# meiji163/bokego

Hardware: AMD Instinct MI355X
Metric: leaf-evals/sec (policy+value, batched 9x9 positions) (higher is better)
Workload: dtype f32; 1 GPU; configs[1]: batch=4096 9x9 positions, PolicyNet logits+softmax and ValueNet, device-resident inputs/outputs; batch_per_gpu=4096, weights=policy_19 + value_synth (tests/golden), precision=f32

## Files before the change

bokego_amd/csrc/bk_engine.cpp:

```cpp
#include <hip/hip_runtime.h>
#include <dlfcn.h>

#include <algorithm>
#include <cmath>
#include <cstdio>
#include <cstdlib>
#include <cstring>
#include <atomic>
#include <chrono>
#include <condition_variable>
#include <mutex>
#include <new>
#include <string>
#include <thread>
#include <vector>

#include "../../include/bokego_amd.h"
#include "../../include/bokego_tree.h"
#include "bk_internal.h"

namespace {

thread_local std::string g_create_error;

// ... 158 lines not shown
    int64_t next_ticket = 1;
    std::string err;
    bk_stats_t st{};
    bool profiling = false;
    std::mutex ev_m;
    struct TimedLaunch { hipEvent_t start, stop; double host_ms; bool ticket; };
    std::vector<TimedLaunch> ev_ring;
    size_t ev_head = 0, ev_pending = 0;
    hipEvent_t epoch = nullptr;
    std::chrono::steady_clock::time_point epoch_host;
    unsigned int* h_redo = nullptr;
    unsigned int* h_redo_dev = nullptr;
    unsigned int redo_seen[BK_DEV_FLAGS] = {};
    bk_plan_opts plan;
    int no_direct = 0, no_head_part = 0, encode_overlap = 0, copy_threads = 6, no_fuse_encode = 0;
    int direct_rows = 1024;
#ifdef BK_TEST_HOOKS
    int fault_at = 0, fault_seen = 0, fault_submit = 0, coop_fault = 0;
#endif
    unsigned int* d_dev_flag = nullptr;
    unsigned int dev_seq = 0;
    float* d_coop_xchg = nullptr;
    unsigned int* d_coop_sync = nullptr;
    unsigned long long* d_stamps = nullptr;
};

namespace {

int fail(bk_engine* e, int code, const std::string& msg) {
    if (e) e->err = msg; else g_create_error = msg;
// ... 9 lines not shown
inline bool inject_fault(bk_engine*) { return false; }
#endif
inline void bump(uint64_t& c, uint64_t v = 1) { __atomic_fetch_add(&c, v, __ATOMIC_RELAXED); }
#define HIP_TRY(e, call)                                                                       \
    do {                                                                                       \
        hipError_t _s = inject_fault(e) ? hipErrorUnknown : (call);                            \
        if (_s != hipSuccess)                                                                  \
            return fail(e, _s == hipErrorOutOfMemory ? BK_ERR_OOM : BK_ERR_HIP,                \
                        std::string(#call) + ": " + hipGetErrorString(_s));                    \
    } while (0)

bool trunk_ok(const bk_trunk_weights& t) {
    for (int l = 0; l < 7; ++l)
        if (!t.conv_w[l] || !t.conv_b[l] || !t.bn_w[l] || !t.bn_b[l] || !t.bn_mean[l] || !t.bn_var[l]) return false;
    return t.head_w && t.head_b;
}

void pack_trunk(const bk_trunk_weights& t, std::vector<float>& wfrag, std::vector<float>& bias) {
    wfrag.assign(BK_WFRAG_FLOATS + BK_WFRAG_PAD_FLOATS, 0.f);
    bias.assign(7 * 128, 0.f);
    size_t base = 0;
    for (int l = 0; l < 7; ++l) {
        const int K = l == 0 ? 5 : 3, cin = l == 0 ? 27 : 128, G = l == 0 ? 2 : 8, TAPS = K * K;
        std::vector<double> scale(128);
        for (int co = 0; co < 128; ++co) scale[co] = (double)t.bn_w[l][co] / std::sqrt((double)t.bn_var[l][co] + kBnEps);
        auto out_ch = [&](int slot) { return l == 6 ? slot : bk_slot_perm(slot); };
        for (int sl = 0; sl < 128; ++sl) {
            const int co = out_ch(sl);
            bias[l * 128 + sl] = (float)(((double)t.conv_b[l][co] - (double)t.bn_mean[l][co]) * scale[co] + (double)t.bn_b[l][co]);
        }
        for (int tp = 0; tp < TAPS; ++tp)
            for (int g = 0; g < G; ++g)
                for (int ct = 0; ct < 8; ++ct)
                    for (int lane = 0; lane < 64; ++lane)
                        for (int j = 0; j < 4; ++j) {
                            const int co = out_ch(16 * ct + (lane & 15)), kq = lane >> 4;
                            int ci = bk_slot_perm(16 * g + 4 * kq + j);
                            if (l == 0 && g == 1) ci = j < 2 ? ci : (j == 2 && kq < 3 ? 24 + kq : cin);
                            float v = 0.f;
                            if (ci < cin) v = (float)((double)t.conv_w[l][((size_t)co * cin + ci) * TAPS + tp] * scale[co]);
                            wfrag[base + ((((size_t)tp * G + g) * 8 + ct) * 64 + lane) * 4 + j] = v;
                        }
        base += (size_t)TAPS * G * 2048;
    }
}

constexpr float kSa16 = 16.f;
void pack_trunk16(const bk_trunk_weights& t, std::vector<_Float16>& wfrag, std::vector<float>& bias16, float* cscale) {
    wfrag.assign(BK16_WFRAG_HALFS + BK16_WFRAG_PAD_HALFS, (_Float16)0.f);
    bias16.assign(7 * 128, 0.f);
    size_t base = 0;
    for (int l = 0; l < 7; ++l) {
        const int K = l == 0 ? 5 : 3, cin = l == 0 ? 27 : 128, S = l == 0 ? 2 : 8, TAPS = K * K;
// ... 29 lines not shown
}

template <typename T>
int upload(bk_engine* e, const std::vector<T>& h, const T** out, std::vector<void*>& fresh) {
    void* d = nullptr;
    HIP_TRY(e, hipMalloc(&d, h.size() * sizeof(T)));
    fresh.push_back(d);
    HIP_TRY(e, hipMemcpy(d, h.data(), h.size() * sizeof(T), hipMemcpyHostToDevice));
    *out = static_cast<const T*>(d);
    return BK_OK;
}

int setup_trunk(bk_engine* e, const bk_trunk_weights& t, bk_net_params& np, double head_scale, double head_shift, std::vector<void*>& fresh) {
    std::vector<float> wfrag, bias, hw(128), hb(81);
    pack_trunk(t, wfrag, bias);
    for (int c = 0; c < 128; ++c) hw[c] = (float)((double)t.head_w[c] * head_scale);
    for (int q = 0; q < 81; ++q) hb[q] = (float)((double)t.head_b[q] * head_scale + head_shift);
    std::vector<_Float16> w16;
    std::vector<float> b16;
    pack_trunk16(t, w16, b16, np.cscale16);
    np.inv_sa16 = 1.f / kSa16;
    int rc;
    if ((rc = upload(e, wfrag, &np.wfrag, fresh))) return rc;
    if ((rc = upload(e, bias, &np.bias, fresh))) return rc;
    if ((rc = upload(e, hw, &np.head_w, fresh))) return rc;
    if ((rc = upload(e, hb, &np.head_b, fresh))) return rc;
    if ((rc = upload(e, w16, &np.wfrag16, fresh))) return rc;
    if ((rc = upload(e, b16, &np.bias16, fresh))) return rc;
    return BK_OK;
}
// ... 165 lines not shown
    }
    return pl;
}

int enqueue(bk_engine* e, const void* d_feats, int dtype, int B, int n_policy, int want, float* d_logits,
            float* d_probs, float* d_values, hipStream_t stream, int precision, unsigned int* d_flag,
            unsigned int tag = 1, bool gated_redo = false, bool allow_coop = false, int lo = 0, int hi = -1) {
    if (B == 0) return BK_OK;
    if (hi < 0) hi = B;
    const bool whole = lo == 0 && hi == B;
    bk_eval_args a{};
    a.net[0] = e->net[0];
    a.net[1] = e->net[1];
    a.feats = d_feats;
    a.feats_dtype = dtype;
    const int np_all = (want & (BK_WANT_LOGITS | BK_WANT_PROBS)) ? n_policy : 0;
    a.off_p = std::min(lo, np_all);
    a.B_policy = std::min(hi, np_all);
    a.off_v = (want & BK_WANT_VALUE) ? lo : 0;
    a.B_value = (want & BK_WANT_VALUE) ? hi : 0;
    a.logits = (want & BK_WANT_LOGITS) ? d_logits : nullptr;
    a.probs = (want & BK_WANT_PROBS) ? d_probs : nullptr;
    a.values = (want & BK_WANT_VALUE) ? d_values : nullptr;
    const int cnt_p = a.B_policy - a.off_p, cnt_v = a.B_value - a.off_v;
    if (cnt_p + cnt_v == 0) return BK_OK;
#ifdef BK_STAMPS
    a.stamps = e->d_stamps;
#endif
    bool timed = false;
    size_t slot = 0;
// ... 100 lines not shown
    if (!e) return fail(nullptr, BK_ERR_OOM, "host allocation failed");
    e->device = device_id;
    e->max_batch = max_batch;
    e->has_policy = policy != nullptr;
    e->has_value = value != nullptr;
    e->precision = BK_PRECISION_F32;
    if (const char* pz = env_str("BK_PRECISION")) e->precision = std::string(pz) == "f16x2" ? BK_PRECISION_F16X2 : BK_PRECISION_F32;
    e->plan.force_nb = env_int("BK_FORCE_NB", 0);
    e->plan.no_split = env_str("BK_NO_SPLIT") != nullptr;
    e->plan.coop = env_int("BK_COOP", -1);
    e->plan.coop3 = env_int("BK_COOP3", -1);
    e->no_direct = env_str("BK_NO_DIRECT") != nullptr;
    e->no_head_part = env_str("BK_NO_HEAD_PART") != nullptr;
    e->encode_overlap = env_str("BK_ENCODE_OVERLAP") != nullptr;
    e->no_fuse_encode = env_str("BK_NO_FUSE_ENCODE") != nullptr;
    e->direct_rows = env_int("BK_DIRECT_ROWS", 1024);
    e->copy_threads = env_int("BK_COPY_THREADS", 6);
    (void)roctx();
    int rc = BK_OK;
    auto bail = [&](int code) {
        g_create_error = e->err;
        bk_engine_destroy(e);
        return code;
    };
#define TRY_CREATE(call)                                                        \
    do {                                                                        \
        hipError_t _s = (call);                                                 \
        if (_s != hipSuccess) {                                                 \
            e->err = std::string(#call) + ": " + hipGetErrorString(_s);         \
            return bail(_s == hipErrorOutOfMemory ? BK_ERR_OOM : BK_ERR_HIP);   \
// ... 430 lines not shown
                exe = bk_mfma_flop_per_workgroup(3) * (pl.head_p + pl.head_v) +
                      bk_mfma_flop_per_workgroup(pl.tail_nb) * (wgs(n_policy - 3 * pl.head_p, pl.tail_nb) + wgs(n_value - 3 * pl.head_v, pl.tail_nb));
                launches = 2;
            } else {
                exe = bk_mfma_flop_per_workgroup(pl.nb1) * (wgs(n_policy, pl.nb1) + wgs(n_value, pl.nb1));
                launches = 1;
            }
        }
    }
    if (executed_mfma_flop) *executed_mfma_flop = exe;
    if (algorithmic_flop) *algorithmic_flop = alg;
    if (n_launches) *n_launches = launches;
    return BK_OK;
}

int bk_has_test_hooks(void) {
#ifdef BK_TEST_HOOKS
    return 1;
#else
    return 0;
#endif
}

namespace {
int* option_field(bk_engine* e, const std::string& n) {
    if (n == "force_nb") return &e->plan.force_nb;
    if (n == "no_split") return &e->plan.no_split;
    if (n == "coop") return &e->plan.coop;
    if (n == "coop3") return &e->plan.coop3;
    if (n == "no_direct") return &e->no_direct;
    if (n == "no_head_part") return &e->no_head_part;
    if (n == "encode_overlap") return &e->encode_overlap;
    if (n == "no_fuse_encode") return &e->no_fuse_encode;
    if (n == "direct_rows") return &e->direct_rows;
    if (n == "copy_threads") return &e->copy_threads;
#ifdef BK_TEST_HOOKS
    if (n == "coop_fault") return &e->coop_fault;
    if (n == "fault_submit") return &e->fault_submit;
#endif
    return nullptr;
}
}

int bk_engine_set_option(bk_engine* e, const char* name, int value) {
    if (!e || !name) return BK_ERR_ARG;
    int* f = option_field(e, name);
    if (!f) return fail(e, BK_ERR_ARG, std::string("unknown engine option '") + name + "'");
    const std::string n = name;
// ... 64 lines not shown
```

bokego_amd/csrc/bk_internal.h:

```cpp
#pragma once
#include <hip/hip_runtime.h>
#include <stdint.h>

#define BK_L0_FLOATS (25 * 2 * 2048)
#define BK_L3_FLOATS (9 * 8 * 2048)
#define BK_WFRAG_FLOATS (BK_L0_FLOATS + 6 * BK_L3_FLOATS)
#define BK_WFRAG_PAD_FLOATS 16384

#define BK16_L0_STEPS 52
#define BK16_L0_HALFS (BK16_L0_STEPS * 4096)
#define BK16_L3_HALFS (72 * 4096)
#define BK16_WFRAG_HALFS (BK16_L0_HALFS + 6 * BK16_L3_HALFS)
#define BK16_WFRAG_PAD_HALFS (4 * 4096)

#define BK_PRECISION_F32 0
#define BK_PRECISION_F16X2 1

#define BK_FEATS_F32_ 0
#define BK_FEATS_U8_ 1
#define BK_FEATS_POS_ 2

struct bk_net_params {
    const float* wfrag;
    const float* bias;
    const float* head_w;
    const float* head_b;
    const float* lin1_wt;
    const float* lin1_b;
    const float* lin2_w;
    float lin2_b;
    const _Float16* wfrag16;
    const float* bias16;
    float cscale16[7];
    float inv_sa16;
};

struct bk_eval_args {
    bk_net_params net[2];
    const void* feats;
    int feats_dtype;
    int B_policy;
    int B_value;
    int off_p, off_v;
    int tasks_p, tasks_v;
    float* logits;
    float* probs;
    float* values;
    unsigned int* overflow;
    unsigned int overflow_tag;
    unsigned int* gate;
    unsigned int* gate_counter;
    unsigned int gate_tag;
    int gate_count;
    float* coop_xchg;
    unsigned int* coop_sync;
    unsigned int* coop_err;
    unsigned int coop_tag;
    int coop_fault;
    unsigned long long* stamps;
// ... 42 lines not shown
```

bokego_amd/csrc/bk_kernels.hip:

```cpp
#include <hip/hip_runtime.h>
#include <stdint.h>
#include <stdlib.h>

#include <type_traits>
#include <utility>

#include "bk_encode_dev.h"
#include "bk_internal.h"

typedef float f32x16 __attribute__((ext_vector_type(16)));
typedef float f32x4 __attribute__((ext_vector_type(4)));
typedef unsigned int u32x4 __attribute__((ext_vector_type(4)));
typedef __attribute__((address_space(3))) const char lds_cchar;
typedef __attribute__((address_space(3))) const f32x4 lds_cf32x4;


#ifndef BK_EXP
#define BK_EXP 0
#endif
#ifdef BK_STAMPS
#define STAMP(k)                                                                                   \
    do {                                                                                           \
        __builtin_amdgcn_sched_barrier(0);                                                         \
        unsigned long long _t;                                                                     \
// ... 54 lines not shown
}
template <int NB>
struct Tiles {
    static_assert(NB >= 1 && NB <= 3, "tiles are laid out for 1-, 2- and 3-board workgroups");
    static constexpr int WM = NB == 3 ? 2 : 1;
    static constexpr int WN = 8 / WM;
    static constexpr int RT = NB == 3 ? 8 : NB == 2 ? 11 : 6;
    static constexpr int CTW = 8 / WN;
    static constexpr int A0 = NB == 3 ? 1 : NB == 2 ? 2 : 0, A1 = NB == 3 ? 6 : NB == 2 ? 9 : 4;
    static constexpr int X0 = NB == 1 ? -1 : 0, X1 = NB == 2 ? 1 : -1;
    static constexpr int Y0a = NB == 3 ? 6 : NB == 2 ? 9 : 4, Y0b = NB == 3 ? 8 : NB == 2 ? 10 : 5, Y1 = NB == 2 ? 10 : NB == 1 ? 5 : -1;
    static constexpr bool WM_EDGES = NB == 3;
    static constexpr bool FRONT = false;
    static constexpr bool DB2 = NB != 3;
    static constexpr int RING = 4;
};
struct TileRow { int b, y, x; bool valid; };
template <int NB>
constexpr TileRow tile_row(int wm, int rt, int p16) {
    TileRow r{0, 4, 0, true};
    if constexpr (NB == 1) {
        if (rt <= 2) {
            const int i = rt * 16 + p16;
            r.y = 1 + i / 7; r.x = 1 + i % 7;
        } else if (rt == 3) {
            if (p16 < 14) { r.y = 1 + p16 % 7; r.x = p16 < 7 ? 0 : 8; }
            else if (p16 == 14) { r.y = 7; r.x = 7; }
            else r.valid = false;
        } else {
            if (p16 < 9) { r.y = rt == 4 ? 0 : 8; r.x = p16; } else r.valid = false;
// ... 38 lines not shown
        for (int rt = 0; rt < Tiles<NB>::RT; ++rt)
            for (int p = 0; p < 16; ++p) {
                const TileRow r = tile_row<NB>(wm, rt, p);
                const int i = (wm * Tiles<NB>::RT + rt) * 16 + p;
                t.a0[i] = Geo<NB>::addr0(r.b, r.y, r.x) - 2 * RP0 - 2 * REC0;
                t.a3v[i] = (Geo<NB>::addr3(r.b, r.y, r.x) - RP3 - REC3) | (r.valid ? 1 : 0);
            }
    return t;
}
template <int NB>
__device__ const RowTable<NB> g_rows = make_row_table<NB>();
__device__ __forceinline__ int in_slot(int c) {
    return c < 24 ? (c & ~15) | ((c & 1) << 3) | (c & 4) | (((c >> 3) & 1) << 1) | ((c >> 1) & 1) : 16 + 4 * (c - 24) + 2;
}

template <class F, bool FIRST>
__device__ __forceinline__ void conv_layer(const char* actb, const float* __restrict__ wl, f32x4 (&acc)[F::CTW][F::RT], int lane,
                                           int wm, int tile0, lds_cchar* (&ap)[F::RT], f32x4 (&W)[F::RING][F::CTW]) {
    constexpr int RT = F::RT, CTW = F::CTW, RING = F::RING;
    static_assert(RING == 4 || RING == 8, "layer 0's 50 groups leave the ring at slot 2: what the 3x3 layers start from");
    constexpr int PH = FIRST ? 0 : 50 % RING;
    constexpr int KW = FIRST ? 5 : 3, TAPS = KW * KW;
    constexpr int HALF = FIRST ? 12 : 5;
    constexpr int G = FIRST ? 2 : 8;
    constexpr int REC = FIRST ? REC0 : REC3, RP = FIRST ? RP0 : RP3;
    (void)actb;
    f32x4 part[CTW][RT];
#pragma unroll
    for (int rt = 0; rt < RT; ++rt) {
#pragma unroll
        for (int ct = 0; ct < CTW; ++ct) acc[ct][rt] = f32x4{0.f, 0.f, 0.f, 0.f};
    }

    const __amdgpu_buffer_rsrc_t wr = __builtin_amdgcn_make_buffer_rsrc(const_cast<float*>(wl + tile0 * 256), 0, 0x7ffffff0, 0x00020000);
// ... 10 lines not shown
        boff += 8192;
    };
    f32x4 A0[RT], A1[RT];
    auto read_a = [&](f32x4& dst, int rt, int imm) {
#if BK_EXP & 1
        (void)dst; (void)rt; (void)imm;
#else
        dst = *reinterpret_cast<lds_cf32x4*>(ap[rt] + imm);
#endif
    };
#if BK_EXP & 1
#pragma unroll
    for (int rt = 0; rt < RT; ++rt) { A0[rt] = f32x4{1.f, 2.f, 3.f, 4.f} * (float)lane; A1[rt] = f32x4{.5f, .25f, .125f, 1.f} * (float)lane; }
#endif

    auto do_group = [&](auto DBc, auto GIc, f32x4 (&Wc)[CTW], f32x4 (&Wn)[CTW], int delta, bool sx0, bool sx1, bool sy0, bool sy1) {
        constexpr bool DB = decltype(DBc)::value;
        constexpr int g = decltype(GIc)::value;
        constexpr int JN = (FIRST && g == 1) ? 3 : 4;
        f32x4 (&Ac)[RT] = (DB && (g & 1)) ? A1 : A0;
        f32x4 (&An)[RT] = (DB && !(g & 1)) ? A1 : A0;
        auto mfmas = [&](int j0, int j1, auto T0, auto T1, auto&& after) {
#pragma unroll
            for (int j = j0; j < j1; ++j)
#pragma unroll
                for (int rt = decltype(T0)::value; rt < decltype(T1)::value; ++rt) {
#pragma unroll
                    for (int ct = 0; ct < CTW; ++ct)
                        acc[ct][rt] = __builtin_amdgcn_mfma_f32_16x16x4f32(Wc[ct][j], Ac[rt][j], acc[ct][rt], 0, 0, 0);
                    after(j, rt);
                }
        };
        auto next_a = [&](int rt) {
            if (g == G - 1) {
// ... 45 lines not shown
            if constexpr (F::X0 >= 0) range(!sx0, std::integral_constant<int, F::X0>{}, std::integral_constant<int, F::X0 + 1>{});
            if constexpr (F::X1 >= 0) range(!sx1, std::integral_constant<int, F::X1>{}, std::integral_constant<int, F::X1 + 1>{});
            if constexpr (F::Y0a >= 0) range(!sy0, std::integral_constant<int, F::Y0a>{}, std::integral_constant<int, F::Y0b>{});
            if constexpr (F::Y1 >= 0) range(!sy1, std::integral_constant<int, F::Y1>{}, std::integral_constant<int, F::Y1 + 1>{});
            next_a(prev);
        }
    };
    using I0 = std::integral_constant<int, 0>;
    using I1 = std::integral_constant<int, 1>;
    using I2 = std::integral_constant<int, 2>;
    using I3 = std::integral_constant<int, 3>;
    using I4 = std::integral_constant<int, 4>;
    using I5 = std::integral_constant<int, 5>;
    using I6 = std::integral_constant<int, 6>;
    using I7 = std::integral_constant<int, 7>;
    auto tap = [&](auto DBc, auto PHc, int t) {
        const int ky = t / KW, kx = t - ky * KW;
        const int d = t == TAPS - 1 ? 0 : (kx == KW - 1 ? RP - (KW - 1) * REC : REC);
        const bool lo_x = kx < KW / 2, hi_x = kx > KW / 2, lo_y = ky < KW / 2, hi_y = ky > KW / 2;
        const bool sx0 = F::WM_EDGES ? (wm == 0 ? lo_x : hi_x) : lo_x, sx1 = hi_x;
        const bool sy0 = F::WM_EDGES ? (wm == 0 ? lo_y : hi_y) : lo_y, sy1 = hi_y;
        constexpr int P0 = decltype(PHc)::value;
        auto grp = [&](auto GIc) {
            constexpr int g = decltype(GIc)::value;
            do_group(DBc, GIc, W[(P0 + g) % RING], W[(P0 + g + RING - 1) % RING], d, sx0, sx1, sy0, sy1);
        };
        grp(I0{});
        grp(I1{});
        if constexpr (!FIRST) {
            grp(I2{});
            grp(I3{});
            grp(I4{});
            grp(I5{});
            grp(I6{});
            grp(I7{});
        }
    };

#pragma unroll
    for (int rt = 0; rt < RT; ++rt) read_a(A0[rt], rt, 0);
    auto taps = [&](auto DBc, int t0, int t1) {
        if constexpr (FIRST) {
            constexpr int U = RING / 2;
#pragma unroll 1
            for (int t = t0; t < t1; t += U) {
                tap(DBc, std::integral_constant<int, 0>{}, t);
                tap(DBc, std::integral_constant<int, 2>{}, t + 1);
                if constexpr (U == 4) {
                    tap(DBc, std::integral_constant<int, 4>{}, t + 2);
                    tap(DBc, std::integral_constant<int, 6>{}, t + 3);
                }
            }
        } else {
#pragma unroll 1
            for (int t = t0; t < t1; ++t) tap(DBc, std::integral_constant<int, PH>{}, t);
        }
    };
    static_assert(!FIRST || (HALF % (RING / 2) == 0 && (TAPS - 1) % (RING / 2) == 0), "layer 0: 12 + 12 taps in whole turns, then tap 24 at slot 0");
    taps(std::true_type{}, 0, HALF);
#pragma unroll
    for (int rt = 0; rt < RT; ++rt)
#pragma unroll
        for (int ct = 0; ct < CTW; ++ct) {
            part[ct][rt] = acc[ct][rt];
            acc[ct][rt] = f32x4{0.f, 0.f, 0.f, 0.f};
        }
    using DB2 = std::integral_constant<bool, F::DB2>;
    taps(DB2{}, HALF, FIRST ? TAPS - 1 : TAPS);
    if constexpr (FIRST) tap(DB2{}, std::integral_constant<int, 0>{}, TAPS - 1);
#pragma unroll
    for (int rt = 0; rt < RT; ++rt) {
        ap[rt] -= (KW - 1) * (RP + REC);
#pragma unroll
        for (int ct = 0; ct < CTW; ++ct) acc[ct][rt] = part[ct][rt] + acc[ct][rt];
    }
}

template <class F>
__device__ __forceinline__ void store_layer(char* actb, const f32x4 (&acc)[F::CTW][F::RT],
                                                 const f32x4 (&bv)[F::CTW], lds_cchar* const (&ap)[F::RT], int store_c,
                                                 unsigned valid, int dummy_byte) {
#pragma unroll
    for (int rt = 0; rt < F::RT; ++rt) {
        typedef __attribute__((address_space(3))) char lds_char;
// ... 10 lines not shown
template <class F>
__device__ __forceinline__ void load_bias(f32x4 (&bv)[F::CTW], const float* __restrict__ bias, int wn, int kq) {
#pragma unroll
    for (int ct = 0; ct < F::CTW; ++ct) bv[ct] = *reinterpret_cast<const f32x4*>(bias + 16 * (F::CTW * wn + ct) + 4 * kq);
}

__device__ __forceinline__ float wave_max(float v) {
#pragma unroll
    for (int o = 32; o > 0; o >>= 1) v = fmaxf(v, __shfl_xor(v, o, 64));
    return v;
}
__device__ __forceinline__ float wave_sum(float v) {
#pragma unroll
    for (int o = 32; o > 0; o >>= 1) v += __shfl_xor(v, o, 64);
    return v;
}

template <int NB, int THREADS>
__device__ __forceinline__ void stage_positions(const bk_eval_args& a, char* actb, int b0, int nb, int tid) {
    using G = Geo<NB>;
    static_assert(THREADS >= 256, "the encoder's mapping: one thread per board point of up to three boards");
    constexpr int SCRATCH = (G::L0_BYTES + 15) & ~15;
    static_assert(SCRATCH + (int)sizeof(bk_enc::EncLds) <= G::L3_BYTES, "the encoder's records live behind the layer-0 input");
    bk_enc::EncLds& S = *reinterpret_cast<bk_enc::EncLds*>(actb + SCRATCH);
    for (int i = tid; i < G::L0_BYTES / 16; i += THREADS) reinterpret_cast<f32x4*>(actb)[i] = f32x4{0.f, 0.f, 0.f, 0.f};
    unsigned char v[27];
    bool live;
    int p, q;
    bk_enc::encode_points(static_cast<const unsigned char*>(a.feats) + (size_t)b0 * BK_POS_BYTES, nb, tid, S, v, live, p, q);
    if (live) {
        const int y = q / 9, x = q - 9 * y;
        char* rec = actb + G::addr0(p, y, x);
#pragma unroll
        for (int c = 0; c < 27; ++c) *reinterpret_cast<float*>(rec + in_slot(c) * 4) = (float)v[c];
    }
}

template <int NB, int THREADS>
__device__ __forceinline__ void stage_input(const bk_eval_args& a, char* actb, int b0, int nb, int tid) {
    using G = Geo<NB>;
    if (a.feats_dtype == BK_FEATS_POS_) {
        stage_positions<NB, THREADS>(a, actb, b0, nb, tid);
        return;
    }
    constexpr int PER = (NB * 2187 + THREADS - 1) / THREADS;
    const int n = nb * 2187;
    float v[PER];
    if (a.feats_dtype == BK_FEATS_F32_) {
        const float* X = static_cast<const float*>(a.feats) + (size_t)b0 * 2187;
// ... 2 lines not shown
            const int e = tid + THREADS * k;
            v[k] = __builtin_nontemporal_load(X + (e < n ? e : 0));
        }
    } else {
        const uint8_t* X = static_cast<const uint8_t*>(a.feats) + (size_t)b0 * 2187;
        uint8_t raw[PER];
#pragma unroll
        for (int k = 0; k < PER; ++k) {
            const int e = tid + THREADS * k;
            raw[k] = __builtin_nontemporal_load(X + (e < n ? e : 0));
        }
#pragma unroll
        for (int k = 0; k < PER; ++k) v[k] = (float)raw[k];
    }
    STAMP_T(t_issued);
    for (int i = tid; i < G::L0_BYTES / 16; i += THREADS) reinterpret_cast<f32x4*>(actb)[i] = f32x4{0.f, 0.f, 0.f, 0.f};
    STAMP_T(t_zeroed);
    __syncthreads();
    STAMP_T(t_barrier);
#pragma unroll
    for (int k = 0; k < PER; ++k) {
        const int e = tid + THREADS * k;
        if (e < n) {
            const int b = e / 2187, ee = e - b * 2187, c = ee / 81, q = ee - c * 81, y = q / 9, x = q - 9 * y;
            *reinterpret_cast<float*>(actb + G::addr0(b, y, x) + in_slot(c) * 4) = v[k];
        }
    }
    STAMP_T(t_scattered);
#ifdef BK_STAMPS
    if (a.stamps && (tid & 63) == 0 && (tid >> 6) < 4)
        a.stamps[((size_t)blockIdx.x * 4 + (tid >> 6)) * 32 + 31] = ((t_zeroed - t_issued) & 0xffff) | (((t_barrier - t_zeroed) & 0xffff) << 16) |
                                                                   (((t_scattered - t_barrier) & 0xffff) << 32);
#endif
}

template <class G>
__device__ __forceinline__ void run_heads(const bk_eval_args& a, const bk_net_params& P, const char* actb, float* hv,
                                              int net, int lane, int board, int bg) {
    float s[2];
#pragma unroll
    for (int k = 0; k < 2; ++k) {
        const int q = lane + 64 * k;
// ... 77 lines not shown

    STAMP(0);
    using F = Tiles<NB>;
    const int wm = wave / F::WN, wn = wave - wm * F::WN;
    f32x4 Wr[F::RING][F::CTW];
    {
        const __amdgpu_buffer_rsrc_t wr0 = __builtin_amdgcn_make_buffer_rsrc(const_cast<float*>(P.wfrag + wn * F::CTW * 256), 0, 0x7ffffff0, 0x00020000);
#pragma unroll
        for (int n = 0; n < F::RING - 1; ++n)
#pragma unroll
            for (int ct = 0; ct < F::CTW; ++ct)
                Wr[n][ct] = __builtin_bit_cast(f32x4, __builtin_amdgcn_raw_buffer_load_b128(wr0, lane * 16 + ct * 1024, n * 8192, 0));
    }
    stage_input<NB, G::THREADS>(a, actb, b0, nb, tid);
    __syncthreads();

    STAMP(1);
    constexpr int RT = F::RT;
    const int kq = lane >> 4;
    f32x4 acc[F::CTW][RT];
    lds_cchar* ap3[RT];
    unsigned valid = 0;
    const int store_c = RP3 + REC3 - kq * 16 + (16 * F::CTW * wn + 4 * kq) * 4;
    f32x4 bv[F::CTW];
    const int row_i = wm * RT * 16 + (lane & 15);
    {
        lds_cchar* ap0[RT];
#pragma unroll
        for (int rt = 0; rt < RT; ++rt) ap0[rt] = (lds_cchar*)actb + (g_rows<NB>.a0[row_i + rt * 16] + kq * 16);
        conv_layer<F, true>(actb, P.wfrag, acc, lane, wm, wn * F::CTW, ap0, Wr);
    }
#pragma unroll
    for (int rt = 0; rt < RT; ++rt) {
        const int e = g_rows<NB>.a3v[row_i + rt * 16];
        ap3[rt] = (lds_cchar*)actb + ((e & ~1) + kq * 16);
        valid |= (unsigned)(e & 1) << rt;
    }
    load_bias<F>(bv, P.bias, wn, kq);
    STAMP(2);
    __syncthreads();
    if constexpr (NB == 3) {
        for (int i = tid; i < 38 * (REC3 / 16); i += G::THREADS) {
            const int rec = i / (REC3 / 16), ch = i - rec * (REC3 / 16);
            const int base = rec < 10 ? rec * REC3 : rec < 37 ? (rec - 9) * RP3 : G::NROWS3 * RP3;
            *reinterpret_cast<f32x4*>(actb + base + ch * 16) = f32x4{0.f, 0.f, 0.f, 0.f};
// ... 24 lines not shown
    if (wave < nb) run_heads<G>(a, P, actb, hs + wave * 96, net, lane, wave, b0 + wave);
    STAMP(30);
}

template <int SC, int SR, int RH>
struct CoopTiles {
    static_assert((SC == 1 || SC == 2 || SC == 4 || SC == 8) && (SR == 1 || SR == 3) && (6 / SR) % RH == 0 && SC * SR > 1,
                  "SC slices of 128/SC output channels x SR slices of 6/SR position tiles");
    static constexpr int S = SC * SR;
    static constexpr int ROWT = 6 / SR;
    static constexpr int RT = ROWT / RH, CTW = 1;
    static constexpr bool SKIP = SR == 1 && RH == 2;
    static constexpr int A0 = 0, A1 = SKIP ? 2 : RT, X0 = -1, X1 = -1, Y0a = SKIP ? 2 : -1, Y0b = SKIP ? 3 : -1, Y1 = -1;
    static constexpr bool WM_EDGES = SKIP, DB2 = true;
    static constexpr int RING = 4;
    static constexpr int tile(int sr, int k) {
        constexpr int PAIRS[6] = {0, 1, 2, 4, 3, 5};
        constexpr int HALVES[6] = {0, 1, 4, 2, 3, 5};
        return SKIP ? HALVES[k] : SR == 3 ? PAIRS[2 * sr + k] : k;
    }
    static constexpr int owner(int q) {
        const int y = q / 9, x = q - 9 * y;
        const int i = (y - 1) * 7 + (x - 1);
        const int t = y == 0 ? 4 : y == 8 ? 5 : (x == 0 || x == 8 || i >= 48) ? 3 : i / 16;
        constexpr int SR_OF[6] = {0, 0, 1, 2, 1, 2};
        return SR == 3 ? SR_OF[t] : 0;
    }
    static constexpr int CT = 8 / SC;
    static constexpr int NW = CT * RH, THREADS = 64 * NW;
    static constexpr bool FRONT = RT == 1;
// ... 30 lines not shown
    f32x4 Wr[F::RING][1];
    {
        const __amdgpu_buffer_rsrc_t wr0 = __builtin_amdgcn_make_buffer_rsrc(const_cast<float*>(P.wfrag + wn * 256), 0, 0x7ffffff0, 0x00020000);
#pragma unroll
        for (int n = 0; n < F::RING - 1; ++n)
            Wr[n][0] = __builtin_bit_cast(f32x4, __builtin_amdgcn_raw_buffer_load_b128(wr0, lane * 16, n * 8192, 0));
    }
    if (tid == 0) {
        const bool poisoned = __hip_atomic_load(a.coop_sync + BK_COOP_POISON_WORD, __ATOMIC_RELAXED, __HIP_MEMORY_SCOPE_AGENT) != 0;
        if (poisoned) __hip_atomic_store(a.coop_err, a.coop_tag, __ATOMIC_RELAXED, __HIP_MEMORY_SCOPE_SYSTEM);
        dead = poisoned;
    }
    STAMP(0);
    stage_input<1, THREADS>(a, actb, bg, 1, tid);
    __syncthreads();
    STAMP(1);

    const int kq = lane >> 4;
    f32x4 acc[1][RT];
    lds_cchar *ap0[RT], *ap3[RT];
    int storea[RT], xoff[RT];
#pragma unroll
    for (int rt = 0; rt < RT; ++rt) {
        const TileRow fr = tile_row<1>(0, F::tile(sr, rh * RT + rt), lane & 15);
        ap0[rt] = (lds_cchar*)actb + (G::addr0(0, fr.y, fr.x) - 2 * RP0 - 2 * REC0 + kq * 16);
        ap3[rt] = (lds_cchar*)actb + (G::addr3(0, fr.y, fr.x) - RP3 - REC3 + kq * 16);
        storea[rt] = fr.valid ? G::addr3(0, fr.y, fr.x) + (16 * wn + 4 * kq) * 4 : dummy_byte;
        xoff[rt] = fr.valid ? (9 * fr.y + fr.x) * 128 + 16 * wn + 4 * kq : -1;
    }
    f32x4 bv[1];
// ... 57 lines not shown
        }
#pragma unroll
        for (int k = 0; k < PER; ++k) {
            const int i = tid + THREADS * k, q = i >> 5, c = i & 31;
            if (foreign(i)) {
                const int y = q / 9, x = q - 9 * y;
                *reinterpret_cast<f32x4*>(actb + G::addr3(0, y, x) + c * 16) = v[k];
            }
        }
        __syncthreads();
        STAMP(5 + 4 * L);
        return true;
    };

    load_bias<F>(bv, P.bias, wn, kq);
    conv_layer<F, true>(actb, P.wfrag, acc, lane, rh, wn, ap0, Wr);
    STAMP(2);
    __syncthreads();
    for (int i = tid; i < G::L3_BYTES / 16; i += THREADS) reinterpret_cast<f32x4*>(actb)[i] = f32x4{0.f, 0.f, 0.f, 0.f};
    __syncthreads();
    exchange(0);
#pragma unroll 1
    for (int L = 1; L < 7; ++L) {
        load_bias<F>(bv, P.bias + L * 128, wn, kq);
        conv_layer<F, false>(actb, P.wfrag + BK_L0_FLOATS + (L - 1) * BK_L3_FLOATS, acc, lane, rh, wn, ap3, Wr);
        STAMP(2 + 4 * L);
        __syncthreads();
        if (!exchange(L)) return;
    }
    if (tid == 0) __hip_atomic_store(cnt, 0u, __ATOMIC_RELAXED, __HIP_MEMORY_SCOPE_AGENT);
    if (wave == 0) run_heads<G>(a, P, actb, hs, net, lane, 0, bg);
// ... 19 lines not shown
    if (tasks == 0) return hipSuccess;
    const int grid = (tasks + 7) / 8 * 8 * S;
    hipLaunchKernelGGL(kern, dim3(grid), dim3(CoopTiles<SC, SR, RH>::THREADS), Geo<1>::LDS_BYTES, stream, args);
    return hipGetLastError();
}

template <int SC>
struct Coop3Tiles {
    static_assert(SC == 2 || SC == 4, "three boards on two or four CUs");
    static constexpr int S = SC, WM = 2, RT = 8, CTW = 1, TB = 0;
    static constexpr int CT = 8 / SC;
    static constexpr int NW = WM * CT, THREADS = 64 * NW;
    static constexpr int A0 = 1, A1 = 6, X0 = 0, X1 = -1, Y0a = 6, Y0b = 8, Y1 = -1;
    static constexpr bool WM_EDGES = true, DB2 = true, FRONT = false;
    static constexpr int RING = 4;
    static constexpr int XCHG_FLOATS = 2 * 243 * 128;
};
static_assert(Coop3Tiles<2>::XCHG_FLOATS * 4 * BK_COOP3_MAX_GROUPS <= BK_COOP_XCHG_BYTES, "exchange buffer");
template <int H>
struct Coop3Tiles8 {
    static constexpr int S = 8, WM = 2, RT = 4, CTW = 1, TB = 4 * H, CT = 1;
    static constexpr int NW = 4, THREADS = 64 * NW;
    static constexpr int A0 = H == 0 ? 1 : 0, A1 = H == 0 ? 4 : 2, X0 = H == 0 ? 0 : -1, X1 = -1;
    static constexpr int Y0a = H == 0 ? -1 : 2, Y0b = H == 0 ? -1 : 4, Y1 = -1;
    static constexpr bool WM_EDGES = true, DB2 = true, FRONT = false;
    static constexpr int RING = 4;
    static constexpr int XCHG_FLOATS = 2 * 243 * 128;
};

template <class F>
__device__ __forceinline__ void coop3_body(const bk_eval_args& a, char* smem, int* dead, int tid, int lane, int wave, int wm, int wn,
                                           int sc, int grp) {
    using G = Geo<3>;
    constexpr int THREADS = F::THREADS, RT = F::RT, S = F::S;
    char* actb = smem;
    const int dummy_byte = G::L3_BYTES;
    float* hs = reinterpret_cast<float*>(smem + G::L3_BYTES) + G::DUMMY_FLOATS;
    const int net = grp >= a.tasks_p;
    const bk_net_params& P = a.net[net];
    const int b0 = (net ? a.off_v + (grp - a.tasks_p) * 3 : a.off_p + grp * 3);
    const int nb = min(3, (net ? a.B_value : a.B_policy) - b0);
// ... 3 lines not shown
    f32x4 Wr[F::RING][1];
    {
        const __amdgpu_buffer_rsrc_t wr0 = __builtin_amdgcn_make_buffer_rsrc(const_cast<float*>(P.wfrag + wn * 256), 0, 0x7ffffff0, 0x00020000);
#pragma unroll
        for (int n = 0; n < F::RING - 1; ++n)
            Wr[n][0] = __builtin_bit_cast(f32x4, __builtin_amdgcn_raw_buffer_load_b128(wr0, lane * 16, n * 8192, 0));
    }
    if (tid == 0) {
        const bool poisoned = __hip_atomic_load(a.coop_sync + BK_COOP_POISON_WORD, __ATOMIC_RELAXED, __HIP_MEMORY_SCOPE_AGENT) != 0;
        if (poisoned) __hip_atomic_store(a.coop_err, a.coop_tag, __ATOMIC_RELAXED, __HIP_MEMORY_SCOPE_SYSTEM);
        *dead = poisoned;
    }
    STAMP(0);
    stage_input<3, THREADS>(a, actb, b0, nb, tid);
    __syncthreads();
    STAMP(1);

    const int kq = lane >> 4;
    f32x4 acc[1][RT];
    lds_cchar* ap3[RT];
    unsigned valid = 0;
    int xoff[RT];
    const int store_c = RP3 + REC3 - kq * 16 + (16 * wn + 4 * kq) * 4;
    f32x4 bv[1];
    const int row_i = (wm * 8 + F::TB) * 16 + (lane & 15);
    {
        lds_cchar* ap0[RT];
#pragma unroll
        for (int rt = 0; rt < RT; ++rt) ap0[rt] = (lds_cchar*)actb + (g_rows<3>.a0[row_i + rt * 16] + kq * 16);
        conv_layer<F, true>(actb, P.wfrag, acc, lane, wm, wn, ap0, Wr);
        STAMP(2);
    }
#pragma unroll
    for (int rt = 0; rt < RT; ++rt) {
        const int e = g_rows<3>.a3v[row_i + rt * 16];
        ap3[rt] = (lds_cchar*)actb + ((e & ~1) + kq * 16);
        valid |= (unsigned)(e & 1) << rt;
        const TileRow fr = tile_row<3>(wm, F::TB + rt, lane & 15);
        xoff[rt] = fr.valid ? (81 * fr.b + 9 * fr.y + fr.x) * 128 + 16 * wn + 4 * kq : -1;
    }
    load_bias<F>(bv, P.bias, wn, kq);
    __syncthreads();
    for (int i = tid; i < 38 * (REC3 / 16); i += THREADS) {
        const int rec = i / (REC3 / 16), ch = i - rec * (REC3 / 16);
        const int base = rec < 10 ? rec * REC3 : rec < 37 ? (rec - 9) * RP3 : G::NROWS3 * RP3;
// ... 269 lines not shown
```

Measured before the change: 505,100 leaf-evals/s.

## Skip layer-0 MFMA k-step for input planes 24..26 when all zero

Staging now records in an LDS flag whether any of input planes 24-26 is nonzero in the workgroup's positions. When none are, and the packed layer-0 weights are all finite, layer 0 runs a specialised variant that drops the MFMA k-step covering those planes in the second channel group. The non-skip path for the 3-board kernel parks half-layer partial sums in spare LDS to relieve register pressure from having two instantiations. The cost is extra code size, a per-launch flag, and a runtime branch; an env var can disable the skip.

```diff
diff --git a/bokego_amd/csrc/bk_engine.cpp b/bokego_amd/csrc/bk_engine.cpp
--- a/bokego_amd/csrc/bk_engine.cpp
+++ b/bokego_amd/csrc/bk_engine.cpp
@@ -196,6 +196,7 @@
     unsigned int redo_seen[BK_DEV_FLAGS] = {};
     bk_plan_opts plan;
     int no_direct = 0, no_head_part = 0, encode_overlap = 0, copy_threads = 6, no_fuse_encode = 0;
+    int no_l0_skip = 0;
     int direct_rows = 1024;
 #ifdef BK_TEST_HOOKS
     int fault_at = 0, fault_seen = 0, fault_submit = 0, coop_fault = 0;
@@ -235,6 +236,11 @@
     for (int l = 0; l < 7; ++l)
         if (!t.conv_w[l] || !t.conv_b[l] || !t.bn_w[l] || !t.bn_b[l] || !t.bn_mean[l] || !t.bn_var[l]) return false;
     return t.head_w && t.head_b;
+}
+
+int l0_input_plane(int g, int kq, int j) {
+    if (g == 0) return bk_slot_perm(4 * kq + j);
+    return j < 2 ? bk_slot_perm(16 + 4 * kq + j) : (j == 2 && kq < 3 ? 24 + kq : 27);
 }
 
 void pack_trunk(const bk_trunk_weights& t, std::vector<float>& wfrag, std::vector<float>& bias) {
@@ -257,7 +263,7 @@
                         for (int j = 0; j < 4; ++j) {
                             const int co = out_ch(16 * ct + (lane & 15)), kq = lane >> 4;
                             int ci = bk_slot_perm(16 * g + 4 * kq + j);
-                            if (l == 0 && g == 1) ci = j < 2 ? ci : (j == 2 && kq < 3 ? 24 + kq : cin);
+                            if (l == 0) ci = l0_input_plane(g, kq, j);
                             float v = 0.f;
                             if (ci < cin) v = (float)((double)t.conv_w[l][((size_t)co * cin + ci) * TAPS + tp] * scale[co]);
                             wfrag[base + ((((size_t)tp * G + g) * 8 + ct) * 64 + lane) * 4 + j] = v;
@@ -317,6 +323,9 @@
 int setup_trunk(bk_engine* e, const bk_trunk_weights& t, bk_net_params& np, double head_scale, double head_shift, std::vector<void*>& fresh) {
     std::vector<float> wfrag, bias, hw(128), hb(81);
     pack_trunk(t, wfrag, bias);
+    np.l0_nonfinite = 0;
+    for (size_t i = 0; i < (size_t)BK_L0_FLOATS; ++i)
+        if (!std::isfinite(wfrag[i])) np.l0_nonfinite = 1;
     for (int c = 0; c < 128; ++c) hw[c] = (float)((double)t.head_w[c] * head_scale);
     for (int q = 0; q < 81; ++q) hb[q] = (float)((double)t.head_b[q] * head_scale + head_shift);
     std::vector<_Float16> w16;
@@ -512,6 +521,7 @@
     a.net[1] = e->net[1];
     a.feats = d_feats;
     a.feats_dtype = dtype;
+    a.no_l0_skip = e->no_l0_skip;
     const int np_all = (want & (BK_WANT_LOGITS | BK_WANT_PROBS)) ? n_policy : 0;
     a.off_p = std::min(lo, np_all);
     a.B_policy = std::min(hi, np_all);
@@ -642,6 +652,7 @@
     e->no_head_part = env_str("BK_NO_HEAD_PART") != nullptr;
     e->encode_overlap = env_str("BK_ENCODE_OVERLAP") != nullptr;
     e->no_fuse_encode = env_str("BK_NO_FUSE_ENCODE") != nullptr;
+    e->no_l0_skip = env_str("BK_NO_L0_SKIP") != nullptr;
     e->direct_rows = env_int("BK_DIRECT_ROWS", 1024);
     e->copy_threads = env_int("BK_COPY_THREADS", 6);
     (void)roctx();
@@ -1102,6 +1113,11 @@
     return BK_OK;
 }
 
+int bk_l0_weight_plane(int group, int kq, int j) {
+    if (group < 0 || group > 1 || kq < 0 || kq > 3 || j < 0 || j > 3) return -1;
+    return l0_input_plane(group, kq, j);
+}
+
 int bk_has_test_hooks(void) {
 #ifdef BK_TEST_HOOKS
     return 1;
@@ -1120,6 +1136,7 @@
     if (n == "no_head_part") return &e->no_head_part;
     if (n == "encode_overlap") return &e->encode_overlap;
     if (n == "no_fuse_encode") return &e->no_fuse_encode;
+    if (n == "no_l0_skip") return &e->no_l0_skip;
     if (n == "direct_rows") return &e->direct_rows;
     if (n == "copy_threads") return &e->copy_threads;
 #ifdef BK_TEST_HOOKS
diff --git a/bokego_amd/csrc/bk_internal.h b/bokego_amd/csrc/bk_internal.h
--- a/bokego_amd/csrc/bk_internal.h
+++ b/bokego_amd/csrc/bk_internal.h
@@ -29,6 +29,7 @@
     const float* lin1_b;
     const float* lin2_w;
     float lin2_b;
+    int l0_nonfinite;
     const _Float16* wfrag16;
     const float* bias16;
     float cscale16[7];
@@ -43,6 +44,7 @@
     int B_value;
     int off_p, off_v;
     int tasks_p, tasks_v;
+    int no_l0_skip;
     float* logits;
     float* probs;
     float* values;
diff --git a/bokego_amd/csrc/bk_kernels.hip b/bokego_amd/csrc/bk_kernels.hip
--- a/bokego_amd/csrc/bk_kernels.hip
+++ b/bokego_amd/csrc/bk_kernels.hip
@@ -92,6 +92,8 @@
     static constexpr bool FRONT = false;
     static constexpr bool DB2 = NB != 3;
     static constexpr int RING = 4;
+    static constexpr int L0_SKIP = NB == 1 ? 0 : 1;
+    static constexpr int L0_PARK = NB == 3 ? 4 : 0;
 };
 struct TileRow { int b, y, x; bool valid; };
 template <int NB>
@@ -160,10 +162,15 @@
     return c < 24 ? (c & ~15) | ((c & 1) << 3) | (c & 4) | (((c >> 3) & 1) << 1) | ((c >> 1) & 1) : 16 + 4 * (c - 24) + 2;
 }
 
-template <class F, bool FIRST>
+template <class F, bool FIRST, int L0SKIP = 0, int PARK = 0>
 __device__ __forceinline__ void conv_layer(const char* actb, const float* __restrict__ wl, f32x4 (&acc)[F::CTW][F::RT], int lane,
-                                           int wm, int tile0, lds_cchar* (&ap)[F::RT], f32x4 (&W)[F::RING][F::CTW]) {
+                                           int wm, int tile0, lds_cchar* (&ap)[F::RT], f32x4 (&W)[F::RING][F::CTW], char* park = nullptr,
+                                           int park_stride = 0) {
     constexpr int RT = F::RT, CTW = F::CTW, RING = F::RING;
+    static_assert(FIRST || PARK == 0, "only layer 0 has free LDS to park sums in");
+    static_assert(PARK <= CTW * RT, "at most every quad of the first chain");
+    typedef __attribute__((address_space(3))) volatile f32x4 lds_vf32x4;
+    static_assert((FIRST || !L0SKIP) && L0SKIP >= 0 && L0SKIP <= 2, "only layer 0 has a k-step that can be empty");
     static_assert(RING == 4 || RING == 8, "layer 0's 50 groups leave the ring at slot 2: what the 3x3 layers start from");
     constexpr int PH = FIRST ? 0 : 50 % RING;
     constexpr int KW = FIRST ? 5 : 3, TAPS = KW * KW;
@@ -204,10 +211,10 @@
     for (int rt = 0; rt < RT; ++rt) { A0[rt] = f32x4{1.f, 2.f, 3.f, 4.f} * (float)lane; A1[rt] = f32x4{.5f, .25f, .125f, 1.f} * (float)lane; }
 #endif
 
-    auto do_group = [&](auto DBc, auto GIc, f32x4 (&Wc)[CTW], f32x4 (&Wn)[CTW], int delta, bool sx0, bool sx1, bool sy0, bool sy1) {
+    auto do_group = [&](auto DBc, auto C2c, auto GIc, f32x4 (&Wc)[CTW], f32x4 (&Wn)[CTW], int delta, bool sx0, bool sx1, bool sy0, bool sy1) {
         constexpr bool DB = decltype(DBc)::value;
         constexpr int g = decltype(GIc)::value;
-        constexpr int JN = (FIRST && g == 1) ? 3 : 4;
+        constexpr int JN = (FIRST && g == 1) ? (L0SKIP == 2 || (L0SKIP == 1 && decltype(C2c)::value) ? 2 : 3) : 4;
         f32x4 (&Ac)[RT] = (DB && (g & 1)) ? A1 : A0;
         f32x4 (&An)[RT] = (DB && !(g & 1)) ? A1 : A0;
         auto mfmas = [&](int j0, int j1, auto T0, auto T1, auto&& after) {
@@ -283,7 +290,7 @@
     using I5 = std::integral_constant<int, 5>;
     using I6 = std::integral_constant<int, 6>;
     using I7 = std::integral_constant<int, 7>;
-    auto tap = [&](auto DBc, auto PHc, int t) {
+    auto tap = [&](auto DBc, auto C2c, auto PHc, int t) {
         const int ky = t / KW, kx = t - ky * KW;
         const int d = t == TAPS - 1 ? 0 : (kx == KW - 1 ? RP - (KW - 1) * REC : REC);
         const bool lo_x = kx < KW / 2, hi_x = kx > KW / 2, lo_y = ky < KW / 2, hi_y = ky > KW / 2;
@@ -292,7 +299,7 @@
         constexpr int P0 = decltype(PHc)::value;
         auto grp = [&](auto GIc) {
             constexpr int g = decltype(GIc)::value;
-            do_group(DBc, GIc, W[(P0 + g) % RING], W[(P0 + g + RING - 1) % RING], d, sx0, sx1, sy0, sy1);
+            do_group(DBc, C2c, GIc, W[(P0 + g) % RING], W[(P0 + g + RING - 1) % RING], d, sx0, sx1, sy0, sy1);
         };
         grp(I0{});
         grp(I1{});
@@ -308,25 +315,25 @@
 
 #pragma unroll
     for (int rt = 0; rt < RT; ++rt) read_a(A0[rt], rt, 0);
-    auto taps = [&](auto DBc, int t0, int t1) {
+    auto taps = [&](auto DBc, auto C2c, int t0, int t1) {
         if constexpr (FIRST) {
             constexpr int U = RING / 2;
 #pragma unroll 1
             for (int t = t0; t < t1; t += U) {
-                tap(DBc, std::integral_constant<int, 0>{}, t);
-                tap(DBc, std::integral_constant<int, 2>{}, t + 1);
+                tap(DBc, C2c, std::integral_constant<int, 0>{}, t);
+                tap(DBc, C2c, std::integral_constant<int, 2>{}, t + 1);
                 if constexpr (U == 4) {
-                    tap(DBc, std::integral_constant<int, 4>{}, t + 2);
-                    tap(DBc, std::integral_constant<int, 6>{}, t + 3);
+                    tap(DBc, C2c, std::integral_constant<int, 4>{}, t + 2);
+                    tap(DBc, C2c, std::integral_constant<int, 6>{}, t + 3);
                 }
             }
         } else {
 #pragma unroll 1
-            for (int t = t0; t < t1; ++t) tap(DBc, std::integral_constant<int, PH>{}, t);
+            for (int t = t0; t < t1; ++t) tap(DBc, C2c, std::integral_constant<int, PH>{}, t);
         }
     };
     static_assert(!FIRST || (HALF % (RING / 2) == 0 && (TAPS - 1) % (RING / 2) == 0), "layer 0: 12 + 12 taps in whole turns, then tap 24 at slot 0");
-    taps(std::true_type{}, 0, HALF);
+    taps(std::true_type{}, std::false_type{}, 0, HALF);
 #pragma unroll
     for (int rt = 0; rt < RT; ++rt)
 #pragma unroll
@@ -334,9 +341,17 @@
             part[ct][rt] = acc[ct][rt];
             acc[ct][rt] = f32x4{0.f, 0.f, 0.f, 0.f};
         }
+    if constexpr (PARK > 0) {
+#pragma unroll
+        for (int i = 0; i < PARK; ++i) *(lds_vf32x4*)(park + i * park_stride) = part[i % CTW][i / CTW];
+    }
     using DB2 = std::integral_constant<bool, F::DB2>;
-    taps(DB2{}, HALF, FIRST ? TAPS - 1 : TAPS);
-    if constexpr (FIRST) tap(DB2{}, std::integral_constant<int, 0>{}, TAPS - 1);
+    taps(DB2{}, std::true_type{}, HALF, FIRST ? TAPS - 1 : TAPS);
+    if constexpr (FIRST) tap(DB2{}, std::true_type{}, std::integral_constant<int, 0>{}, TAPS - 1);
+    if constexpr (PARK > 0) {
+#pragma unroll
+        for (int i = 0; i < PARK; ++i) part[i % CTW][i / CTW] = *(lds_vf32x4*)(park + i * park_stride);
+    }
 #pragma unroll
     for (int rt = 0; rt < RT; ++rt) {
         ap[rt] -= (KW - 1) * (RP + REC);
@@ -377,6 +392,31 @@
 #pragma unroll
     for (int o = 32; o > 0; o >>= 1) v += __shfl_xor(v, o, 64);
     return v;
+}
+
+template <int NB>
+__device__ __forceinline__ unsigned* l0_live_word(char* actb) {
+    return reinterpret_cast<unsigned*>(actb + Geo<NB>::L3_BYTES + Geo<NB>::DUMMY_FLOATS * 4);
+}
+template <int NB>
+__device__ __forceinline__ bool l0_can_skip(const bk_eval_args& a, const bk_net_params& P, char* actb) {
+    return __builtin_amdgcn_readfirstlane(*l0_live_word<NB>(actb) | (unsigned)a.no_l0_skip | (unsigned)P.l0_nonfinite) == 0;
+}
+template <class F>
+__device__ __forceinline__ void conv_layer0(bool skip, const char* actb, const float* __restrict__ wl, f32x4 (&acc)[F::CTW][F::RT], int lane,
+                                            int wm, int tile0, lds_cchar* (&ap)[F::RT], f32x4 (&W)[F::RING][F::CTW], char* park = nullptr,
+                                            int park_stride = 0) {
+    if constexpr (F::L0_SKIP == 0) {
+        conv_layer<F, true>(actb, wl, acc, lane, wm, tile0, ap, W);
+    } else if (skip) {
+        asm volatile("; layer 0 without the k-step of planes 24..26");
+        conv_layer<F, true, F::L0_SKIP>(actb, wl, acc, lane, wm, tile0, ap, W);
+        asm volatile("; end of layer 0 without the k-step of planes 24..26");
+    } else {
+        asm volatile("; layer 0, every k-step");
+        conv_layer<F, true, 0, F::L0_PARK>(actb, wl, acc, lane, wm, tile0, ap, W, park, park_stride);
+        asm volatile("; end of layer 0, every k-step");
+    }
 }
 
 template <int NB, int THREADS>
@@ -386,6 +426,7 @@
     constexpr int SCRATCH = (G::L0_BYTES + 15) & ~15;
     static_assert(SCRATCH + (int)sizeof(bk_enc::EncLds) <= G::L3_BYTES, "the encoder's records live behind the layer-0 input");
     bk_enc::EncLds& S = *reinterpret_cast<bk_enc::EncLds*>(actb + SCRATCH);
+    if (tid == 0) *l0_live_word<NB>(actb) = 0;
     for (int i = tid; i < G::L0_BYTES / 16; i += THREADS) reinterpret_cast<f32x4*>(actb)[i] = f32x4{0.f, 0.f, 0.f, 0.f};
     unsigned char v[27];
     bool live;
@@ -396,6 +437,7 @@
         char* rec = actb + G::addr0(p, y, x);
 #pragma unroll
         for (int c = 0; c < 27; ++c) *reinterpret_cast<float*>(rec + in_slot(c) * 4) = (float)v[c];
+        if (v[24] | v[25] | v[26]) __hip_atomic_store(l0_live_word<NB>(actb), 1u, __ATOMIC_RELAXED, __HIP_MEMORY_SCOPE_WORKGROUP);
     }
 }
 
@@ -428,18 +470,22 @@
         for (int k = 0; k < PER; ++k) v[k] = (float)raw[k];
     }
     STAMP_T(t_issued);
+    if (tid == 0) *l0_live_word<NB>(actb) = 0;
     for (int i = tid; i < G::L0_BYTES / 16; i += THREADS) reinterpret_cast<f32x4*>(actb)[i] = f32x4{0.f, 0.f, 0.f, 0.f};
     STAMP_T(t_zeroed);
     __syncthreads();
     STAMP_T(t_barrier);
+    unsigned live_bits = 0;
 #pragma unroll
     for (int k = 0; k < PER; ++k) {
         const int e = tid + THREADS * k;
         if (e < n) {
             const int b = e / 2187, ee = e - b * 2187, c = ee / 81, q = ee - c * 81, y = q / 9, x = q - 9 * y;
             *reinterpret_cast<float*>(actb + G::addr0(b, y, x) + in_slot(c) * 4) = v[k];
-        }
-    }
+            if (c >= 24) live_bits |= __float_as_uint(v[k]);
+        }
+    }
+    if (live_bits) __hip_atomic_store(l0_live_word<NB>(actb), 1u, __ATOMIC_RELAXED, __HIP_MEMORY_SCOPE_WORKGROUP);
     STAMP_T(t_scattered);
 #ifdef BK_STAMPS
     if (a.stamps && (tid & 63) == 0 && (tid >> 6) < 4)
@@ -547,6 +593,7 @@
     }
     stage_input<NB, G::THREADS>(a, actb, b0, nb, tid);
     __syncthreads();
+    const bool l0_skip = l0_can_skip<NB>(a, P, actb);
 
     STAMP(1);
     constexpr int RT = F::RT;
@@ -561,7 +608,9 @@
         lds_cchar* ap0[RT];
 #pragma unroll
         for (int rt = 0; rt < RT; ++rt) ap0[rt] = (lds_cchar*)actb + (g_rows<NB>.a0[row_i + rt * 16] + kq * 16);
-        conv_layer<F, true>(actb, P.wfrag, acc, lane, wm, wn * F::CTW, ap0, Wr);
+        constexpr int PARK_BASE = (G::L0_BYTES + 15) & ~15;
+        static_assert(PARK_BASE + F::L0_PARK * G::THREADS * 16 <= G::L3_BYTES, "the parked sums fit between the layer-0 input and the end of the activations");
+        conv_layer0<F>(l0_skip, actb, P.wfrag, acc, lane, wm, wn * F::CTW, ap0, Wr, actb + PARK_BASE + tid * 16, G::THREADS * 16);
     }
 #pragma unroll
     for (int rt = 0; rt < RT; ++rt) {
@@ -616,6 +665,7 @@
     static constexpr int A0 = 0, A1 = SKIP ? 2 : RT, X0 = -1, X1 = -1, Y0a = SKIP ? 2 : -1, Y0b = SKIP ? 3 : -1, Y1 = -1;
     static constexpr bool WM_EDGES = SKIP, DB2 = true;
     static constexpr int RING = 4;
+    static constexpr int L0_SKIP = 2, L0_PARK = 0;
     static constexpr int tile(int sr, int k) {
         constexpr int PAIRS[6] = {0, 1, 2, 4, 3, 5};
         constexpr int HALVES[6] = {0, 1, 4, 2, 3, 5};
@@ -676,6 +726,7 @@
     STAMP(0);
     stage_input<1, THREADS>(a, actb, bg, 1, tid);
     __syncthreads();
+    const bool l0_skip = l0_can_skip<1>(a, P, actb);
     STAMP(1);
 
     const int kq = lane >> 4;
@@ -763,7 +814,7 @@
     };
 
     load_bias<F>(bv, P.bias, wn, kq);
-    conv_layer<F, true>(actb, P.wfrag, acc, lane, rh, wn, ap0, Wr);
+    conv_layer0<F>(l0_skip, actb, P.wfrag, acc, lane, rh, wn, ap0, Wr);
     STAMP(2);
     __syncthreads();
     for (int i = tid; i < G::L3_BYTES / 16; i += THREADS) reinterpret_cast<f32x4*>(actb)[i] = f32x4{0.f, 0.f, 0.f, 0.f};
@@ -813,6 +864,7 @@
     static constexpr int A0 = 1, A1 = 6, X0 = 0, X1 = -1, Y0a = 6, Y0b = 8, Y1 = -1;
     static constexpr bool WM_EDGES = true, DB2 = true, FRONT = false;
     static constexpr int RING = 4;
+    static constexpr int L0_SKIP = 2, L0_PARK = 0;
     static constexpr int XCHG_FLOATS = 2 * 243 * 128;
 };
 static_assert(Coop3Tiles<2>::XCHG_FLOATS * 4 * BK_COOP3_MAX_GROUPS <= BK_COOP_XCHG_BYTES, "exchange buffer");
@@ -824,6 +876,7 @@
     static constexpr int Y0a = H == 0 ? -1 : 2, Y0b = H == 0 ? -1 : 4, Y1 = -1;
     static constexpr bool WM_EDGES = true, DB2 = true, FRONT = false;
     static constexpr int RING = 4;
+    static constexpr int L0_SKIP = 2, L0_PARK = 0;
     static constexpr int XCHG_FLOATS = 2 * 243 * 128;
 };
 
@@ -857,6 +910,7 @@
     STAMP(0);
     stage_input<3, THREADS>(a, actb, b0, nb, tid);
     __syncthreads();
+    const bool l0_skip = l0_can_skip<3>(a, P, actb);
     STAMP(1);
 
     const int kq = lane >> 4;
@@ -871,7 +925,7 @@
         lds_cchar* ap0[RT];
 #pragma unroll
         for (int rt = 0; rt < RT; ++rt) ap0[rt] = (lds_cchar*)actb + (g_rows<3>.a0[row_i + rt * 16] + kq * 16);
-        conv_layer<F, true>(actb, P.wfrag, acc, lane, wm, wn, ap0, Wr);
+        conv_layer0<F>(l0_skip, actb, P.wfrag, acc, lane, wm, wn, ap0, Wr);
         STAMP(2);
     }
 #pragma unroll
```

Result: no change. 508,100 leaf-evals/s (median of 6 runs) (+0.6%).
